# poriya219/modulations

Measured on NVIDIA B200. Metric: turbo_info_throughput_N212_R1/3_8it, higher is better.
Workload: dtype f32/f64

## Files before the change

### modulations_b200/csrc/decode_tpf.cu

```cuda
#include "common.cuh"
#include "tpf_core.cuh"
#include "tpf_dev.cuh"

namespace b200dvb {

namespace {

using namespace tpf;

constexpr int kW = kTpfWin;

__device__ unsigned long long g_tpf_cycles[8];

struct TpfArgs {
    TpfGeom g;
    int B, iterations, n_tiles, n_llr, vec4;
    double sf_inner, sf_last;
    const int16_t *tab;
    const void *llr;
    long long llr_stride;
    int32_t *bits;
    uint32_t *packed;
    const uint8_t *ref_bits;
    unsigned long long *counters;
    unsigned char *ws;
};

constexpr int kRingPairs = 4;
constexpr int kStageBytes = 12288;
constexpr int kRowFloats = kStageBytes / 8;

struct Ctx {
    int N, M, T;
    int f, isb, lane;
    unsigned tq;
    unsigned ycol;
    float4 *srec;
    unsigned char *stage;
    const int16_t *perm, *inv;
    float4 *L1A, *L2A;
    double2 *Le, *LeF, *Yb;
    float4 *CK;
    unsigned long long pol;
    unsigned one;
    __device__ __forceinline__ float4 *wstore() const { return reinterpret_cast<float4 *>(stage); }
    __device__ __forceinline__ float4 *slotZ() const { return reinterpret_cast<float4 *>(stage + 8192); }
    __device__ __forceinline__ float4 *slotX() const { return reinterpret_cast<float4 *>(stage + 10240); }
};

__device__ __forceinline__ void smem_get(const Ctx &c, int k, float (&g)[8])
{
    const float4 lo = c.srec[((k - c.T) * 2) * 16 + c.f], hi = c.srec[((k - c.T) * 2 + 1) * 16 + c.f];
    g[0] = lo.x; g[1] = lo.y; g[2] = lo.z; g[3] = lo.w; g[4] = hi.x; g[5] = hi.y; g[6] = hi.z; g[7] = hi.w;
}
__device__ __forceinline__ void smem_put(const Ctx &c, int k, const float (&g)[8])
{
    c.srec[((k - c.T) * 2) * 16 + c.f] = make_float4(g[0], g[1], g[2], g[3]);
    c.srec[((k - c.T) * 2 + 1) * 16 + c.f] = make_float4(g[4], g[5], g[6], g[7]);
}

struct Buf { float a[8], b[8]; };
template <int KIND> __device__ __forceinline__ void pf_issue(const Ctx &c, int j, Buf &B)
{
    if (KIND == 0) tm_ld8(c.tq + 8u * j, B.a);
    if (KIND == 1) smem_get(c, c.isb ? c.N - 1 - j : j, B.a);
    if (KIND == 2) {
        const unsigned col = 8u * (c.N - 1 - j);
        tm_ld8_half(c.tq + col, B.b);
        tm_ld8_half(c.tq + (16u << 16) + col, B.a);
    }
}
template <int KIND> __device__ __forceinline__ void pf_complete(const Ctx &c, Buf &B, float (&g)[8])
{
    if (KIND == 0) tm_wait_ld(B.a);
    if (KIND == 2) { tm_wait_ld(B.a); tm_wait_ld(B.b); }
#pragma unroll
    for (int i = 0; i < 8; ++i) g[i] = (KIND == 2 && c.isb) ? B.b[i] : B.a[i];
}

__device__ __forceinline__ constexpr int apos(int p) { return (p >> 1) | ((p & 1) << 3); }
__device__ __forceinline__ void pass_out(const Ctx &c, const float (&v)[16], float (&n)[16])
{
#pragma unroll
    for (int p = 0; p < 16; ++p) n[p] = c.isb ? v[rho4(p)] : v[apos(p)];
}
__device__ __forceinline__ void ck_store(const Ctx &c, int slot, const float (&v)[16])
{
    float n[16];
    pass_out(c, v, n);
#pragma unroll
    for (int q = 0; q < 4; ++q)
        st_ws(c.CK + (slot * 4 + q) * 32 + c.lane, make_float4(n[4 * q], n[4 * q + 1], n[4 * q + 2], n[4 * q + 3]));
}

template <int KIND, bool CK>
__device__ __forceinline__ void pass_two(const Ctx &c, int j, int j1, Buf &B0, Buf &B1, float (&g)[8], float (&v)[16])
{
    pf_issue<KIND>(c, j + 1, B1);
    if (CK) ck_store(c, (c.M - j) / kW - 1, v);
    pass_step(v, g, c.isb);
    pf_complete<KIND>(c, B1, g);
    pf_issue<KIND>(c, min(j + 2, j1 - 1), B0);
    pass_step(v, g, c.isb);
    pf_complete<KIND>(c, B0, g);
}
template <int KIND, bool CKA, bool CKB>
__device__ __forceinline__ void pass_loop(const Ctx &c, int j0, int j1, Buf &B0, Buf &B1, float (&g)[8], float (&v)[16])
{
    int j = j0;
    for (; j + 4 <= j1; j += 4) {
        pass_two<KIND, CKA>(c, j, j1, B0, B1, g, v);
        pass_two<KIND, CKB>(c, j + 2, j1, B0, B1, g, v);
    }
    if (j < j1) pass_two<KIND, CKA>(c, j, j1, B0, B1, g, v);
}
template <int KIND, bool CKPT>
__device__ __forceinline__ void run_pass(const Ctx &c, int j0, int j1, float (&v)[16])
{
    static_assert(kW == 4, "checkpoints alternate between the step pairs of a four-step body");
    if (j0 >= j1) return;
    Buf B0, B1;
    float g[8];
    pf_issue<KIND>(c, j0, B0);
    pf_complete<KIND>(c, B0, g);
    if (!CKPT) { pass_loop<KIND, false, false>(c, j0, j1, B0, B1, g, v); return; }
    if (j0 == 0 && (c.M % kW) != 0) ck_store(c, c.M / kW, v);
    if (((c.M - j0) % kW) == 0) pass_loop<KIND, CKPT, false>(c, j0, j1, B0, B1, g, v);
    else                        pass_loop<KIND, false, CKPT>(c, j0, j1, B0, B1, g, v);
}

__device__ __forceinline__ void issue_ckpt(const Ctx &c, int slot)
{
    float4 *dst = (c.isb ? c.slotZ() : c.slotX()) + c.lane;
#pragma unroll
    for (int q = 0; q < 4; ++q) cpa16(dst + q * 32, c.CK + (slot * 4 + q) * 32 + c.lane, c.one);
}
template <bool ALPHA = false>
__device__ __forceinline__ void slot_get(const float4 *slot, int lane, float (&v)[16])
{
    constexpr int P[4] = {ALPHA ? apos(0) : 0, ALPHA ? apos(1) : 1, ALPHA ? apos(2) : 2, ALPHA ? apos(3) : 3};
#pragma unroll
    for (int q = 0; q < 4; ++q) {
        const float4 t = slot[q * 32 + lane];
        const int b = ALPHA ? 2 * q : 4 * q;
        v[b + P[0]] = t.x; v[b + P[1]] = t.y; v[b + P[2]] = t.z; v[b + P[3]] = t.w;
    }
}
template <bool ALPHA = false>
__device__ __forceinline__ void slot_put(float4 *slot, int lane, const float (&v)[16])
{
    constexpr int P[4] = {ALPHA ? apos(0) : 0, ALPHA ? apos(1) : 1, ALPHA ? apos(2) : 2, ALPHA ? apos(3) : 3};
#pragma unroll
    for (int q = 0; q < 4; ++q) {
        const int b = ALPHA ? 2 * q : 4 * q;
        slot[q * 32 + lane] = make_float4(v[b + P[0]], v[b + P[1]], v[b + P[2]], v[b + P[3]]);
    }
}

__device__ __forceinline__ void st256_f64(void *p, double a, double b, double c, double d)
{
    asm volatile("st.global.cg.v4.f64 [%0], {%1,%2,%3,%4};" :: "l"(p), "d"(a), "d"(b), "d"(c), "d"(d) : "memory");
}
__device__ __forceinline__ void ld256_f64(const void *p, double2 &lo, double2 &hi)
{
    asm volatile("ld.global.cg.v4.f64 {%0,%1,%2,%3}, [%4];" : "=d"(lo.x), "=d"(lo.y), "=d"(hi.x), "=d"(hi.y) : "l"(p) : "memory");
}
__device__ __forceinline__ unsigned char *y_entry(const Ctx &c, int k_even)
{
    return reinterpret_cast<unsigned char *>(c.Yb) + ((size_t)(k_even >> 1) * 16 + c.f) * 32;
}
struct YQ { double2 y[kW]; };
__device__ __forceinline__ void yq_load(const Ctx &c, int w0, int len, YQ &q)
{
    static_assert(kW == 4, "two 32-byte entries per window");
    ld256_f64(y_entry(c, w0), q.y[0], q.y[1]);
    ld256_f64(y_entry(c, len > 2 ? w0 + 2 : w0), q.y[2], q.y[3]);
}
__device__ __forceinline__ void yq_park(const Ctx &c, const YQ &q, int w0, int len, int ck_slot)
{

#pragma unroll
    for (int u = 0; u < kW; ++u)
        asm volatile("tcgen05.st.sync.aligned.32x32b.x4.b32 [%0], {%1,%2,%3,%4};"
                     :: "r"(c.tq + c.ycol + 4u * u), "r"(__double2loint(q.y[u].x)), "r"(__double2hiint(q.y[u].x)),
                        "r"(__double2loint(q.y[u].y)), "r"(__double2hiint(q.y[u].y)) : "memory");
    tm_wait_st();
    const int dir = (c.lane >> 3) & 1, pr = (c.lane >> 2) & 1, l16 = c.lane & 15;
    const int w0d = __shfl_sync(0xffffffffu, w0, dir << 4);
    const void *line = c.lane < 16
        ? static_cast<const void *>(reinterpret_cast<const unsigned char *>(c.Yb) + ((size_t)((w0d >> 1) + pr) * 16) * 32 + (c.lane & 3) * 128)
        : static_cast<const void *>(c.CK + (ck_slot * 4 + (l16 >> 2)) * 32 + (l16 & 3) * 8);
    if (c.lane < 16 ? 2 * pr < len : ck_slot >= 0) l2_discard(line);
}

struct Pend { float uv[4], y[4]; int idx; };
__device__ __forceinline__ void pend_flush(const Ctx &c, Pend &p, double sf, double2 *LeOut)
{
    double ea, eb;
    make_extrinsic(p.uv, __hiloint2double(__float_as_int(p.y[1]), __float_as_int(p.y[0])),
                   __hiloint2double(__float_as_int(p.y[3]), __float_as_int(p.y[2])), sf, ea, eb);
    if (p.idx >= 0) st_ws(LeOut + p.idx * 16 + c.f, make_double2(ea, eb));
    p.idx = -1;
}
template <bool TM>
__device__ __forceinline__ void window(const Ctx &c, int wa, int w0, int len, double sf,
                                       double2 *LeOut, int nslot, int nw0, int nlen, Pend &pend)
{
    Buf B;
    auto issue = [&](int u) {
        if (TM) { tm_ld8(c.tq + 8u * (wa + u), B.a); tm_ld8(c.tq + 8u * (wa + len - 1 - u), B.b); }
        else    smem_get(c, w0 + u, B.a);
    };
    auto complete = [&](float (&g)[8]) {
        if (TM) { tm_wait_ld(B.a); tm_wait_ld(B.b); }
#pragma unroll
        for (int i = 0; i < 8; ++i) g[i] = (TM && c.isb) ? B.b[i] : B.a[i];
    };
    YQ nq;
    if (nlen) yq_load(c, nw0, nlen, nq);
    float g[8];
    float4 *ws = c.wstore() + c.lane;
    {
        float Z[16];
        issue(len - 1);
        slot_get(c.slotZ(), c.lane, Z);
        complete(g);
        slot_put(ws + (len - 1) * 128, 0, Z);
        issue(len - 2);
        pend_flush(c, pend, sf, LeOut);
        bwd_step(Z, g);
        complete(g);
        for (int u = len - 2; u >= 0; --u) {
            slot_put(ws + u * 128, 0, Z);
            issue(u > 0 ? u - 1 : 0);
            bwd_step(Z, g);
            complete(g);
        }
        if (!c.isb) slot_put(c.slotZ(), c.lane, Z);
    }
    float X[16];
    slot_get<true>(c.slotX(), c.lane, X);
    if (nslot >= 0) issue_ckpt(c, nslot);
    cpa_commit();
    float yr[4], yn[4], uvp[4], zs[16];
    tm_ld4(c.tq + c.ycol, yr);
    issue(len > 1 ? 1 : 0);
    slot_get(ws, 0, zs);
    ext_step(X, zs, g, uvp);
    tm_wait_ld4(yr);
    complete(g);
    for (int u = 1; u < len; ++u) {
        tm_ld4(c.tq + c.ycol + 4u * u, yn);
        issue(u + 1 < len ? u + 1 : u);
        slot_get(ws + u * 128, 0, zs);
        float uv[4];
        ext_step(X, zs, g, uv);
        double ea, eb;
        make_extrinsic(uvp, __hiloint2double(__float_as_int(yr[1]), __float_as_int(yr[0])),
                       __hiloint2double(__float_as_int(yr[3]), __float_as_int(yr[2])), sf, ea, eb);
        st_ws(LeOut + (w0 + u - 1) * 16 + c.f, make_double2(ea, eb));
        tm_wait_ld4(yn);
        complete(g);
#pragma unroll
        for (int i = 0; i < 4; ++i) { uvp[i] = uv[i]; yr[i] = yn[i]; }
    }
#pragma unroll
    for (int i = 0; i < 4; ++i) { pend.uv[i] = uvp[i]; pend.y[i] = yr[i]; }
    pend.idx = w0 + len - 1;
    if (c.isb) slot_put<true>(c.slotX(), c.lane, X);
    if (nlen) yq_park(c, nq, nw0, nlen, nslot - 1);
}


__device__ __forceinline__ int lpos(const Ctx &c, int k, int fr) { return k < c.M ? k * 32 + fr : (c.N - 1 - k) * 32 + 16 + fr; }

struct Idx { int a, b; };
__device__ __forceinline__ void idx_get(const Ctx &c, int jn, const int16_t *tbl, Idx &x)
{
    jn = min(jn, c.M - 2);
    const int k0 = c.isb ? c.N - 1 - jn : jn, k1 = c.isb ? k0 - 1 : k0 + 1;
    x.a = tbl[k0]; x.b = tbl[k1];
}
__device__ __forceinline__ void prep_load_pair(const Ctx &c, unsigned char *slot, int jn, const float4 *Lsrc,
                                               const Idx &x, bool first)
{
    jn = min(jn, c.M - 2);
    const unsigned d = s_addr(slot) * c.one;
    const float4 *src = Lsrc + jn * 32 + c.lane;
    cpa16_stream_off<0, 0>(d, src, c.pol);
    cpa16_stream_off<1024, 512>(d, src, c.pol);
    if (!first) {
        cpa16_off<512, 0>(d, c.Le + x.a * 16 + c.f);
        cpa16_off<1536, 0>(d, c.Le + x.b * 16 + c.f);
    }
}
struct Raw { float4 xA, xB; double2 laA, laB; };
template <bool FIRST>
__device__ __forceinline__ void raw_get(const unsigned char *slot, Raw &r)
{
    r.xA = *reinterpret_cast<const float4 *>(slot);
    r.xB = *reinterpret_cast<const float4 *>(slot + 1024);
    r.laA = r.laB = make_double2(0.0, 0.0);
    if (!FIRST) {
        r.laA = *reinterpret_cast<const double2 *>(slot + 512);
        r.laB = *reinterpret_cast<const double2 *>(slot + 1536);
    }
}
struct PrepRec { float gA[8], gB[8]; };
__device__ __forceinline__ void prep_pair(const Ctx &c, const Raw &r, int jn, PrepRec &out)
{
    jn = min(jn, c.M - 2);
    const double2 YA = make_double2(d_add((double)r.xA.x, r.laA.x), d_add((double)r.xA.y, r.laA.y));
    const double2 YB = make_double2(d_add((double)r.xB.x, r.laB.x), d_add((double)r.xB.y, r.laB.y));
    make_record(YA.x, YA.y, r.xA.z, r.xA.w, out.gA);
    make_record(YB.x, YB.y, r.xB.z, r.xB.w, out.gB);
#ifndef TPF_ABL_NOY
    const int ke = c.isb ? c.N - 2 - jn : jn;
    st256_f64(y_entry(c, ke), c.isb ? YB.x : YA.x, c.isb ? YB.y : YA.y, c.isb ? YA.x : YB.x, c.isb ? YA.y : YB.y);
#endif
}
struct PrepState { PrepRec r; Raw raw; Idx ix; int ps; };
template <bool FIRST, bool TMST>
__device__ __forceinline__ void pass1a_pair(const Ctx &c, int jj, const float4 *Lsrc, const int16_t *tbl,
// ... 52 lines not shown
}

template <bool FIRST>
__device__ __forceinline__ void pass1a(const Ctx &c, bool second, float (&v)[16])
{
    const float4 *Lsrc = second ? c.L2A : c.L1A;
    const int16_t *tbl = second ? c.perm : c.inv;
    unsigned char *ring = c.stage + c.lane * 16;
    PrepState P;
    P.ix.a = P.ix.b = 0;
#pragma unroll 1
    for (int p = 0; p < kRingPairs; ++p) {
        if (!FIRST) idx_get(c, 2 * p, tbl, P.ix);
        prep_load_pair(c, ring + p * 2048, 2 * p, Lsrc, P.ix, FIRST);
        cpa_commit();
    }
    if (!FIRST) idx_get(c, 2 * kRingPairs, tbl, P.ix);
    cpa_wait<kRingPairs - 1>();
    raw_get<FIRST>(ring, P.raw);
    prep_pair(c, P.raw, 0, P.r);
    prep_load_pair(c, ring, 2 * kRingPairs, Lsrc, P.ix, FIRST);
    cpa_commit();
    if (!FIRST) idx_get(c, 2 * kRingPairs + 2, tbl, P.ix);
    cpa_wait<kRingPairs - 1>();
    raw_get<FIRST>(ring + 2048, P.raw);
    prep_load_pair(c, ring + 2048, 2 * kRingPairs + 2, Lsrc, P.ix, FIRST);
    cpa_commit();
    if (!FIRST) idx_get(c, 2 * kRingPairs + 4, tbl, P.ix);
    P.ps = 2 % kRingPairs;
    pass1a_range<FIRST, true>(c, 0, c.T, Lsrc, tbl, P, v);
    pass1a_range<FIRST, false>(c, c.T, c.M, Lsrc, tbl, P, v);
    cpa_wait<0>();
}

template <bool TIMED>
__device__ __forceinline__ void siso(const Ctx &c, bool second, bool first, bool last, double sf, long long (&ph)[8])
{
    long long tA = TIMED ? clock64() : 0;
    const int N = c.N, M = c.M, T = c.T, lane = c.lane;
    double2 *LeOut = last ? c.LeF : c.Le;
    float v[16];
#pragma unroll
    for (int s = 0; s < 16; ++s) v[s] = 0.f;
    if (first) pass1a<true>(c, second, v);
    else       pass1a<false>(c, second, v);
    tm_wait_st();
    __syncwarp();
    if (!first && !last)
        for (int i = lane; i < N * 2; i += 32) l2_discard(c.Le + i * 8);
    if (TIMED) { const long long t = clock64(); ph[1] += t - tA; tA = t; }
    run_pass<1, false>(c, M, N - T, v);
    run_pass<2, false>(c, N - T, N, v);
    if (TIMED) { const long long t = clock64(); ph[2] += t - tA; tA = t; }
    const int nfull = M / kW, rag = M % kW, nwin = nfull + (rag ? 1 : 0);
    auto win_w0 = [&](int i) { return i < nfull ? (c.isb ? M + i * kW : M - (i + 1) * kW) : (c.isb ? N - rag : 0); };
    auto win_len = [&](int i) { return i < nfull ? kW : rag; };
    {
        YQ q0;
        yq_load(c, win_w0(0), win_len(0), q0);
        run_pass<0, true>(c, 0, T, v);
        run_pass<1, true>(c, T, M, v);
        yq_park(c, q0, win_w0(0), win_len(0), -1);
    }
    if (TIMED) { const long long t = clock64(); ph[3] += t - tA; tA = t; }
    {
        float n[16];
        pass_out(c, v, n);
        slot_put(c.isb ? c.slotZ() : c.slotX(), lane ^ 16, n);
    }
    const int n_inner = (M - T) / kW;
    issue_ckpt(c, 0);
    cpa_commit();
    Pend pend;
#pragma unroll
    for (int i = 0; i < 4; ++i) pend.uv[i] = pend.y[i] = 0.f;
    pend.idx = -1;
    for (int i = 0; i < nwin; ++i) {
        cpa_wait<0>();
        __syncwarp();
        const int wa = i < nfull ? M - (i + 1) * kW : 0;
        const int nlen = i + 1 < nwin ? win_len(i + 1) : 0;
        const int nw0 = i + 1 < nwin ? win_w0(i + 1) : 0;
        if (i < n_inner) window<false>(c, wa, win_w0(i), win_len(i), sf, LeOut, nlen ? i + 1 : -1, nw0, nlen, pend);
        else             window<true>(c, wa, win_w0(i), win_len(i), sf, LeOut, nlen ? i + 1 : -1, nw0, nlen, pend);
        if (TIMED && i == n_inner - 1) { const long long t = clock64(); ph[4] += t - tA; tA = t; }
    }
    pend_flush(c, pend, sf, LeOut);
    cpa_wait<0>();
    __syncwarp();
    if (TIMED) { const long long t = clock64(); ph[5] += t - tA; tA = t; }
}

template <bool TIMED, class LlrT>
__global__ void __launch_bounds__(kTpfWarps * 32, 1)
tpf_kernel(const TpfArgs A)
{
    extern __shared__ __align__(16) unsigned char smem_raw[];
    const TpfGeom g = A.g;
    const int N = g.N;
    const int tid = threadIdx.x, lane = tid & 31, warp = tid >> 5;
    int16_t *tab = reinterpret_cast<int16_t *>(smem_raw);
    const int tab_bytes = ((2 * N * 2 + 15) / 16) * 16;
    unsigned *tmem_slot = reinterpret_cast<unsigned *>(smem_raw + tab_bytes);
    float4 *srec_all = reinterpret_cast<float4 *>(smem_raw + tab_bytes + 64);
    unsigned char *stage_all = reinterpret_cast<unsigned char *>(srec_all + (size_t)kTpfWarps * g.mid * 2 * 16);
    if (warp == 0) {
        asm volatile("tcgen05.alloc.cta_group::1.sync.aligned.shared::cta.b32 [%0], %1;"
                     ::"r"((unsigned)__cvta_generic_to_shared(tmem_slot)), "r"(g.tmem_cols) : "memory");
        asm volatile("tcgen05.relinquish_alloc_permit.cta_group::1.sync.aligned;" ::: "memory");
    }
    for (int i = tid; i < 2 * N; i += blockDim.x) tab[i] = A.tab[i];
    const unsigned mbar = (unsigned)__cvta_generic_to_shared(smem_raw + tab_bytes + 32 + 8 * warp);
    unsigned mphase = 0;
    if (lane == 0) { mbar_init(mbar, 1); mbar_fence_init(); }
    asm volatile("tcgen05.fence::before_thread_sync;" ::: "memory");
    __syncthreads();
    asm volatile("tcgen05.fence::after_thread_sync;" ::: "memory");
    const unsigned tmem_base = *tmem_slot;

    Ctx c;
    c.N = N; c.M = g.M; c.T = g.T;
    c.f = lane & 15; c.isb = lane >> 4; c.lane = lane;
    c.tq = tmem_base + (((unsigned)warp * 32u) << 16);
    c.ycol = 8u * g.T;
    c.srec = srec_all + (size_t)warp * g.mid * 2 * 16;
    {
        volatile unsigned *slots = reinterpret_cast<volatile unsigned *>(smem_raw + tab_bytes);
        if (lane == 0) { slots[4 + warp] = (unsigned)warp * kStageBytes; slots[1] = 1u; }
        __syncwarp();
        c.stage = stage_all + slots[4 + warp];
        c.one = slots[1];
        __syncwarp();
    }
    c.perm = tab; c.inv = tab + N;
    const int wg = blockIdx.x * kTpfWarps + warp;
    unsigned char *ws = A.ws + (size_t)wg * g.ws_per_warp;
    c.L1A = reinterpret_cast<float4 *>(ws + g.off_l1);
    c.L2A = reinterpret_cast<float4 *>(ws + g.off_l2);
    c.Le = reinterpret_cast<double2 *>(ws + g.off_le);
    c.LeF = reinterpret_cast<double2 *>(ws + g.off_lef);
    c.Yb = reinterpret_cast<double2 *>(ws + g.off_y);
    c.CK = reinterpret_cast<float4 *>(ws + g.off_ck);
    asm volatile("createpolicy.fractional.L2::evict_first.b64 %0, 1.0;" : "=l"(c.pol));
    const int16_t *g_off = A.tab + 2 * N;

    unsigned long long bit_err = 0, frm_err = 0, frames_done = 0;
    long long ph[8] = {0, 0, 0, 0, 0, 0, 0, 0};
    const long long t_begin = TIMED ? clock64() : 0;
    for (int tile = wg; tile < A.n_tiles; tile += gridDim.x * kTpfWarps) {
        const long long frame0 = (long long)tile * kTpfFrames;
        const long long t0 = TIMED ? clock64() : 0;
        if (A.vec4) {
            const int nq = llr_row_q<LlrT>(A.n_llr);
            const int pitch4 = ((nq + 6) & ~7) + 1;
            const int rec_bytes = g.mid * 2 * 16 * (int)sizeof(float4);
            const bool in_rec = rec_bytes > kStageBytes;
            float4 *rowbuf = in_rec ? c.srec : reinterpret_cast<float4 *>(c.stage);
            const int fit = (in_rec ? rec_bytes : kStageBytes - N * 16) / (pitch4 * 16);
            const int lg = fit >= 8 ? 3 : fit >= 4 ? 2 : 1, G = 1 << lg, KQ = 32 >> lg;
            const int fr = lane & (G - 1), kq = lane >> lg;
            int4 *otab = reinterpret_cast<int4 *>(in_rec ? c.stage : c.stage + G * pitch4 * 16);
            for (int k = lane; k < N; k += 32) {
                const unsigned oa = (unsigned short)__ldg(g_off + k), op = (unsigned short)__ldg(g_off + c.perm[k]);
                const unsigned o0 = (unsigned short)__ldg(g_off + N + k), o1 = (unsigned short)__ldg(g_off + 2 * N + k);
                const unsigned o2 = (unsigned short)__ldg(g_off + 3 * N + k), o3 = (unsigned short)__ldg(g_off + 4 * N + k);
                otab[k] = make_int4((int)(oa | (op << 16)), (int)(o0 | (o1 << 16)), (int)(o2 | (o3 << 16)), 0);
            }
            auto pull = [&](int g0) {
                if (lane == 0) {
                    int live_rows = 0;
                    for (int r = 0; r < G; ++r) live_rows += frame0 + g0 + r < A.B;
                    fence_proxy_async();
                    mbar_expect_tx(mbar, (unsigned)(live_rows * nq * 16));
                    for (int r = 0; r < live_rows; ++r)
                        bulk_g2s_stream(rowbuf + r * pitch4, static_cast<const LlrT *>(A.llr) + (frame0 + g0 + r) * A.llr_stride, (unsigned)(nq * 16), mbar, c.pol);
                }
            };
            pull(0);
            if (A.ref_bits) {
                const int lines = (2 * N * kTpfFrames + 127) / 128;
                const long long nb = min((long long)kTpfFrames, A.B - frame0) * 2 * N;
                for (int i = lane; i < lines; i += 32)
                    if ((long long)i * 128 < nb) asm volatile("prefetch.global.L2 [%0];" ::"l"(A.ref_bits + frame0 * 2 * N + i * 128));
            }
            const LlrT *row = reinterpret_cast<const LlrT *>(rowbuf + fr * pitch4);
            for (int g0 = 0; g0 < kTpfFrames; g0 += G) {
                mbar_wait(mbar, mphase);
                mphase ^= 1u;
                const bool livef = frame0 + g0 + fr < A.B;
#pragma unroll 4
                for (int k0 = 0; k0 < N; k0 += KQ) {
                    const int k = k0 + kq;
                    const int4 e = otab[min(k, N - 1)];
                    const int oa = (short)(e.x & 0xffff), op = e.x >> 16, o0 = (short)(e.y & 0xffff), o1 = e.y >> 16;
                    const int o2 = (short)(e.z & 0xffff), o3 = e.z >> 16;
                    float4 x1 = make_float4(0.f, 0.f, 0.f, 0.f), x2 = x1;
                    if (livef) {
                        x1.x = llr_f32(row[oa]); x1.y = llr_f32(row[oa + 1]); x2.x = llr_f32(row[op]); x2.y = llr_f32(row[op + 1]);
                        if (o0 >= 0) x1.z = llr_f32(row[o0]);
                        if (o1 >= 0) x1.w = llr_f32(row[o1]);
                        if (o2 >= 0) x2.z = llr_f32(row[o2]);
                        if (o3 >= 0) x2.w = llr_f32(row[o3]);
                    }
// ... 60 lines not shown
                for (int t = 0; t < 8; ++t) {
                    const int k = min(kb + t, N - 1);
                    const unsigned dt = d + t * 512;
                    cpa16_off<0, 0>(dt, c.L1A + lpos(c, k, c.f));
                    cpa16_off<4096, 0>(dt, c.LeF + c.inv[k] * 16 + c.f);
                    cpa16_off<8192, 0>(dt, c.Le + k * 16 + c.f);
                }
            }
            cpa_commit();
        };
        int any_err = 0;
        unsigned word = 0;
        for (int b = 0; b < nst; ++b) hissue(b, b);
        for (int b = 0, st = 0; b < nbu; ++b) {
            if (nst == 3) cpa_wait<2>(); else if (nst == 2) cpa_wait<1>(); else cpa_wait<0>();
            const int kb = (c.isb + 2 * (b >> 1)) * 16 + 8 * (b & 1);
            const unsigned char *src = hbuf + st * kHB + lane * 16;
            unsigned short rb[8];
#pragma unroll
            for (int t = 0; t < 8; ++t) rb[t] = *reinterpret_cast<const unsigned short *>(refp + 2 * min(kb + t, N - 1));
#pragma unroll
            for (int t = 0; t < 8; ++t) {
                const int k = kb + t;
                const float4 ab = *reinterpret_cast<const float4 *>(src + t * 512);
                const double2 la = *reinterpret_cast<const double2 *>(src + 4096 + t * 512);
                const double2 e1 = *reinterpret_cast<const double2 *>(src + 8192 + t * 512);
                const double LA = d_add(d_add((double)ab.x, la.x), e1.x);
                const double LB = d_add(d_add((double)ab.y, la.y), e1.y);
                const int bA = LA < 0.0, bB = LB < 0.0;
                if (k < N) {
                    word |= (unsigned)(bA | (bB << 1)) << (2 * (8 * (b & 1) + t));
                    if (live && A.bits)
                        *reinterpret_cast<int2 *>(A.bits + (size_t)frame * 2 * N + 2 * k) = make_int2(bA, bB);
                    if (cnt) {
                        const int errs = (bA != (rb[t] & 0xff)) + (bB != (rb[t] >> 8));
                        bit_err += errs;
                        any_err |= errs;
                    }
                }
            }
            hissue(b + nst, st);
            st = st + 1 == nst ? 0 : st + 1;
            if (b & 1) {
                const int w = c.isb + b - 1;
                if (live && A.packed && w < nwords) A.packed[(size_t)frame * wpf + w] = word;
                word = 0;
            }
        }
        cpa_wait<0>();
        any_err |= __shfl_xor_sync(0xffffffffu, any_err, 16);
        if (live && !c.isb) { frames_done += 1; frm_err += any_err ? 1 : 0; }
        __syncwarp();
        if (TIMED) ph[6] += clock64() - t6;
    }
    if (TIMED && lane == 0) {
        ph[7] = clock64() - t_begin;
        for (int i = 0; i < 8; ++i) atomicAdd(&g_tpf_cycles[i], (unsigned long long)ph[i]);
    }
    if (A.counters) {
        for (int o = 16; o > 0; o >>= 1) {
            bit_err += __shfl_xor_sync(0xffffffffu, bit_err, o);
            frm_err += __shfl_xor_sync(0xffffffffu, frm_err, o);
            frames_done += __shfl_xor_sync(0xffffffffu, frames_done, o);
        }
        if (lane == 0) {
            if (bit_err) atomicAdd(A.counters + 0, bit_err);
            if (frm_err) atomicAdd(A.counters + 1, frm_err);
            if (frames_done) {
                atomicAdd(A.counters + 2, frames_done);
                atomicAdd(A.counters + 3, frames_done * 2ull * N);
            }
        }
    }
    asm volatile("tcgen05.fence::before_thread_sync;" ::: "memory");
    __syncthreads();
    if (warp == 0)
        asm volatile("tcgen05.dealloc.cta_group::1.sync.aligned.b32 %0, %1;" ::"r"(tmem_base), "r"(g.tmem_cols) : "memory");
}

}

int tpf_configure(Codec &c)
{
    TpfGeom &g = c.tpf;
    g = TpfGeom{};
    const int N = c.N;
    if (N < 16 || (N % 4) != 0) return B200DVB_OK;
    const int M = N / 2;
    int T = M < 64 ? M : 64;
    while (T > 0 && (((M - T) % kW) != 0 || 8 * T + 4 * kW > 512)) --T;
    if (T < kW) return B200DVB_OK;
    g.N = N; g.M = M; g.T = T; g.mid = N - 2 * T;
    g.nfull = M / kW; g.rag = M % kW; g.nslots = g.nfull + (g.rag ? 1 : 0);
    g.tmem_cols = 32;
    while (g.tmem_cols < 8 * T + 4 * kW) g.tmem_cols *= 2;
    if (g.tmem_cols > 512) return B200DVB_OK;
    const size_t tab_bytes = ((size_t)2 * N * 2 + 15) / 16 * 16;
    g.smem_bytes = tab_bytes + 64 + (size_t)kTpfWarps * g.mid * 2 * 16 * sizeof(float4) + (size_t)kTpfWarps * kStageBytes;
    int dev = 0;
    cudaDeviceProp prop;
    B2_CUDA(cudaGetDevice(&dev));
    B2_CUDA(cudaGetDeviceProperties(&prop, dev));
    if (g.smem_bytes > (size_t)prop.sharedMemPerBlockOptin) return B200DVB_OK;
    size_t off = 0;
    auto take = [&](size_t bytes) { const size_t o = off; off += (bytes + 255) / 256 * 256; return o; };
    g.off_l1 = take((size_t)N * 16 * sizeof(float4));
    g.off_l2 = take((size_t)N * 16 * sizeof(float4));
    g.off_le = take((size_t)N * 16 * sizeof(double2));
    g.off_lef = take((size_t)N * 16 * sizeof(double2));
    g.off_y = take((size_t)N * 16 * sizeof(double2));
    g.off_ck = take((size_t)g.nslots * 4 * 32 * sizeof(float4));
    g.ws_per_warp = off;
    B2_CUDA(cudaFuncSetAttribute(tpf_kernel<false, float>, cudaFuncAttributeMaxDynamicSharedMemorySize, (int)prop.sharedMemPerBlockOptin));
    B2_CUDA(cudaFuncSetAttribute(tpf_kernel<true, float>, cudaFuncAttributeMaxDynamicSharedMemorySize, (int)prop.sharedMemPerBlockOptin));
    B2_CUDA(cudaFuncSetAttribute(tpf_kernel<false, __half>, cudaFuncAttributeMaxDynamicSharedMemorySize, (int)prop.sharedMemPerBlockOptin));
    B2_CUDA(cudaFuncSetAttribute(tpf_kernel<true, __half>, cudaFuncAttributeMaxDynamicSharedMemorySize, (int)prop.sharedMemPerBlockOptin));
    g.enabled = 1;
    return B200DVB_OK;
}

int tpf_read_phase_cycles(double *out_h, int reset)
{
    unsigned long long h[8];
    B2_CUDA(cudaMemcpyFromSymbol(h, g_tpf_cycles, sizeof h));
    for (int i = 0; i < 8; ++i) out_h[i] = (double)h[i];
    if (reset) {
        unsigned long long z[8] = {0, 0, 0, 0, 0, 0, 0, 0};
        B2_CUDA(cudaMemcpyToSymbol(g_tpf_cycles, z, sizeof z));
    }
    return B200DVB_OK;
}

static int tpf_grid(const Codec &c, int B)
{
    const int tiles = (B + kTpfFrames - 1) / kTpfFrames;
    const int ctas = (tiles + kTpfWarps - 1) / kTpfWarps;
    return ctas < c.num_sms ? ctas : c.num_sms;
}

size_t tpf_workspace_bytes(const Codec &c, int B)
{
    return (size_t)tpf_grid(c, B) * kTpfWarps * c.tpf.ws_per_warp + 256;
}

template <class LlrT> static void tpf_start(const TpfArgs &A, bool timed, int grid, size_t smem, cudaStream_t s)
{
// ... 35 lines not shown
```

### modulations_b200/csrc/common.cuh

```cuda
#pragma once
#include <cuda_runtime.h>
#include <cuda_fp16.h>
#include <stdint.h>
#include <stddef.h>
#include "../../include/b200dvb.h"

namespace b200dvb {

__device__ __forceinline__ float llr_f32(float x) { return x; }
__device__ __forceinline__ float llr_f32(__half x) { return __half2float(x); }
template <class L> __device__ __forceinline__ float llr_ldg(const L *p) { return llr_f32(__ldg(p)); }
__device__ __forceinline__ float2 llr_ldg2(const float *p) { return __ldg(reinterpret_cast<const float2 *>(p)); }
__device__ __forceinline__ float2 llr_ldg2(const __half *p) { return __half22float2(__ldg(reinterpret_cast<const __half2 *>(p))); }
template <class L> __host__ __device__ __forceinline__ int llr_row_q(int n) { return sizeof(L) == 4 ? (n + 3) / 4 : (n + 7) / 8; }
template <class K32, class K16>
inline cudaError_t occupancy_both_formats(int *occ, K32 k32, K16 k16, int threads, size_t smem)
{
    int a = 0, b = 0;
    cudaError_t e = cudaOccupancyMaxActiveBlocksPerMultiprocessor(&a, k32, threads, smem);
    if (e == cudaSuccess) e = cudaOccupancyMaxActiveBlocksPerMultiprocessor(&b, k16, threads, smem);
    *occ = a < b ? a : b;
    return e;
}

void set_cuda_error(cudaError_t e, const char *where);
#define B2_CUDA(call)                                                     \
    do {                                                                  \
        cudaError_t e__ = (call);                                         \
        if (e__ != cudaSuccess) {                                         \
            ::b200dvb::set_cuda_error(e__, #call);                        \
            return B200DVB_ECUDA;                                         \
        }                                                                 \
    } while (0)

constexpr int kMaxN = 2048;

constexpr int kFramesPerCta = 8;
constexpr int kCtaThreads = 64;
constexpr int kMaxGroups = 7;
constexpr int kMaxCtaThreads = 448;
constexpr int kWin = 8;

struct QuadGeom {
    int N;
    unsigned magic;
    int M;
    int nckA;
    int nckB;
    int rec_stride;
    int ck_stride;
    int groups;
    int threads;
    int use_tmem;
    int tmem_cols;
    int y_slots;
    int frames;
    int ctas_per_sm;
    int grec;
    size_t smem_bytes;
};

constexpr int kTpfFrames = 16;
constexpr int kTpfWarps = 4;
constexpr int kTpfWin = 4;

struct TpfGeom {
    int enabled;
    int N, M;
    int T;
    int mid;
    int nfull, rag;
    int nslots;
    int tmem_cols;
    size_t smem_bytes;
    size_t off_l1, off_l2, off_le, off_lef, off_y, off_ck, off_init;
    size_t ws_per_warp;
};

struct Codec {
    int N = 0, period = 0, iterations = 0, n_llr = 0;
    double sf_inner = 0.7, sf_last = 1.0;
    QuadGeom geom{};
    QuadGeom geom_g{};
    TpfGeom tpf{};
    TpfGeom nii{};
    int num_sms = 0;
    int vec_ab = 0, vec_wy = 0;
    int opt_kernel = 0;
    int opt_no_row_staging = 0;
    int opt_phase_timers = 0;
    int lat_pad = 0;
    int lat_enabled = 0, lat_frames_per_wave = 0;
    int opt_mode = 0;
    int16_t *d_tab = nullptr;
    int32_t next_state[64], out_W[64], out_Y[64];
    int32_t circ_lut[16];
    int16_t *h_tab = nullptr;
};

struct Modem {
    int mod_id = 0, bps = 0, M = 0;
    int separable = 0;
    int half = 0, nlev = 0;
    int pwl = 0;
    int nseg = 0;
    float pwl_x0[2] = {0, 0}, pwl_invd[2] = {0, 0};
    double *d_table64 = nullptr;
    float *d_table32 = nullptr;
    float *d_pwl = nullptr;
    double h_table[512];
};

int launch_decode(const Codec &c, int B, const void *llr, bool f16, long long llr_stride, int32_t *bits,
                  uint32_t *packed, const uint8_t *ref_bits, unsigned long long *counters,
                  void *ws, size_t ws_bytes, cudaStream_t s);
int launch_siso(const Codec &c, int B, const float *Lc_A, const float *Lc_B, const float *Lc_W,
                const float *Lc_Y, const double *La_A, const double *La_B, double sf,
                double *Le_A, double *Le_B, void *ws, size_t ws_bytes, cudaStream_t s);
size_t decode_workspace_bytes(const Codec &c, int B);
size_t siso_workspace_bytes(const Codec &c, int B);
int quad_configure(Codec &c);
int tpf_configure(Codec &c);
int tpf_launch_decode(const Codec &c, int B, const void *llr, bool f16, long long llr_stride, int32_t *bits,
                      uint32_t *packed, const uint8_t *ref_bits, unsigned long long *counters,
// ... 46 lines not shown
```

Baseline: 4.061.

## Add register-resident full-window decode path and per-tile counter flush with ablation hooks

```diff
diff --git a/modulations_b200/csrc/decode_tpf.cu b/modulations_b200/csrc/decode_tpf.cu
--- a/modulations_b200/csrc/decode_tpf.cu
+++ b/modulations_b200/csrc/decode_tpf.cu
@@ -193,13 +193,30 @@
     if (c.lane < 16 ? 2 * pr < len : ck_slot >= 0) l2_discard(line);
 }
 
-struct Pend { float uv[4], y[4]; int idx; };
+struct Pend { float uv[4], y[4]; int idx; unsigned sink; };
+__device__ __forceinline__ void out_epilogue(const float (&uv)[4], const float (&y)[4], double sf, double &ea, double &eb)
+{
+#ifndef TPF_ABL_OUT_FP64
+    make_extrinsic(uv, __hiloint2double(__float_as_int(y[1]), __float_as_int(y[0])),
+                   __hiloint2double(__float_as_int(y[3]), __float_as_int(y[2])), sf, ea, eb);
+#else
+    ea = __hiloint2double(__float_as_int(uv[1]) ^ __float_as_int(y[1]), __float_as_int(uv[0]) ^ __float_as_int(y[0]));
+    eb = __hiloint2double(__float_as_int(uv[3]) ^ __float_as_int(y[3]), __float_as_int(uv[2]) ^ __float_as_int(y[2]));
+#endif
+}
+__device__ __forceinline__ void out_store(const Ctx &c, double2 *LeOut, int k, double ea, double eb, unsigned &sink)
+{
+#ifndef TPF_ABL_OUT_LE
+    st_ws(LeOut + k * 16 + c.f, make_double2(ea, eb));
+#else
+    sink ^= (unsigned)__double2loint(ea) ^ (unsigned)__double2hiint(ea) ^ (unsigned)__double2loint(eb) ^ (unsigned)__double2hiint(eb);
+#endif
+}
 __device__ __forceinline__ void pend_flush(const Ctx &c, Pend &p, double sf, double2 *LeOut)
 {
     double ea, eb;
-    make_extrinsic(p.uv, __hiloint2double(__float_as_int(p.y[1]), __float_as_int(p.y[0])),
-                   __hiloint2double(__float_as_int(p.y[3]), __float_as_int(p.y[2])), sf, ea, eb);
-    if (p.idx >= 0) st_ws(LeOut + p.idx * 16 + c.f, make_double2(ea, eb));
+    out_epilogue(p.uv, p.y, sf, ea, eb);
+    if (p.idx >= 0) out_store(c, LeOut, p.idx, ea, eb, p.sink);
     p.idx = -1;
 }
 template <bool TM>
@@ -216,22 +233,35 @@
 #pragma unroll
         for (int i = 0; i < 8; ++i) g[i] = (TM && c.isb) ? B.b[i] : B.a[i];
     };
+#ifdef TPF_ABL_OUT_REC2
+    auto issue2 = [&](int) {};
+    auto complete2 = [&](float (&)[8]) {};
+#else
+    auto issue2 = issue;
+    auto complete2 = complete;
+#endif
     YQ nq;
+#ifndef TPF_ABL_OUT_GLUE
     if (nlen) yq_load(c, nw0, nlen, nq);
+#endif
     float g[8];
     float4 *ws = c.wstore() + c.lane;
+    float Z[16];
     {
-        float Z[16];
         issue(len - 1);
         slot_get(c.slotZ(), c.lane, Z);
         complete(g);
+#ifndef TPF_ABL_OUT_BETA
         slot_put(ws + (len - 1) * 128, 0, Z);
+#endif
         issue(len - 2);
         pend_flush(c, pend, sf, LeOut);
         bwd_step(Z, g);
         complete(g);
         for (int u = len - 2; u >= 0; --u) {
+#ifndef TPF_ABL_OUT_BETA
             slot_put(ws + u * 128, 0, Z);
+#endif
             issue(u > 0 ? u - 1 : 0);
             bwd_step(Z, g);
             complete(g);
@@ -240,33 +270,115 @@
     }
     float X[16];
     slot_get<true>(c.slotX(), c.lane, X);
+#ifndef TPF_ABL_OUT_GLUE
     if (nslot >= 0) issue_ckpt(c, nslot);
     cpa_commit();
+#endif
     float yr[4], yn[4], uvp[4], zs[16];
+#ifndef TPF_ABL_OUT_Y
     tm_ld4(c.tq + c.ycol, yr);
-    issue(len > 1 ? 1 : 0);
+#else
+#pragma unroll
+    for (int i = 0; i < 4; ++i) yr[i] = yn[i] = pend.y[i];
+#endif
+    issue2(len > 1 ? 1 : 0);
+#ifndef TPF_ABL_OUT_BETA
     slot_get(ws, 0, zs);
+#else
+#pragma unroll
+    for (int i = 0; i < 16; ++i) zs[i] = Z[i];
+#endif
     ext_step(X, zs, g, uvp);
+#ifndef TPF_ABL_OUT_Y
     tm_wait_ld4(yr);
-    complete(g);
+#endif
+    complete2(g);
     for (int u = 1; u < len; ++u) {
+#ifndef TPF_ABL_OUT_Y
         tm_ld4(c.tq + c.ycol + 4u * u, yn);
-        issue(u + 1 < len ? u + 1 : u);
+#endif
+        issue2(u + 1 < len ? u + 1 : u);
+#ifndef TPF_ABL_OUT_BETA
         slot_get(ws + u * 128, 0, zs);
+#endif
         float uv[4];
         ext_step(X, zs, g, uv);
         double ea, eb;
-        make_extrinsic(uvp, __hiloint2double(__float_as_int(yr[1]), __float_as_int(yr[0])),
-                       __hiloint2double(__float_as_int(yr[3]), __float_as_int(yr[2])), sf, ea, eb);
-        st_ws(LeOut + (w0 + u - 1) * 16 + c.f, make_double2(ea, eb));
+        out_epilogue(uvp, yr, sf, ea, eb);
+        out_store(c, LeOut, w0 + u - 1, ea, eb, pend.sink);
+#ifndef TPF_ABL_OUT_Y
         tm_wait_ld4(yn);
-        complete(g);
+#endif
+        complete2(g);
 #pragma unroll
         for (int i = 0; i < 4; ++i) { uvp[i] = uv[i]; yr[i] = yn[i]; }
     }
 #pragma unroll
     for (int i = 0; i < 4; ++i) { pend.uv[i] = uvp[i]; pend.y[i] = yr[i]; }
     pend.idx = w0 + len - 1;
+    if (c.isb) slot_put<true>(c.slotX(), c.lane, X);
+#ifndef TPF_ABL_OUT_GLUE
+    if (nlen) yq_park(c, nq, nw0, nlen, nslot - 1);
+#endif
+}
+
+__device__ __forceinline__ void window_full(const Ctx &c, int wa, int w0, double sf,
+                                            double2 *LeOut, int nslot, int nw0, int nlen, Pend &pend)
+{
+    constexpr int L = kW;
+    YQ nq;
+    if (nlen) yq_load(c, nw0, nlen, nq);
+    float4 *ws = c.wstore() + c.lane;
+    float r[L][8], Z[L][16], Zt[16];
+    {
+        float t[L][8];
+#pragma unroll
+        for (int u = 0; u < L; ++u) tm_ld8(c.tq + 8u * (wa + u), t[u]);
+        slot_get(c.slotZ(), c.lane, Zt);
+        slot_put(ws, 0, Zt);
+        pend_flush(c, pend, sf, LeOut);
+#pragma unroll
+        for (int u = 0; u < L; ++u) tm_wait_ld(t[u]);
+#pragma unroll
+        for (int u = 0; u < L; ++u)
+#pragma unroll
+            for (int i = 0; i < 8; ++i) r[u][i] = c.isb ? t[L - 1 - u][i] : t[u][i];
+    }
+#pragma unroll
+    for (int u = L - 1; u >= 0; --u) {
+#pragma unroll
+        for (int s = 0; s < 16; ++s) Z[u][s] = u == L - 1 ? Zt[s] : Z[u + 1][s];
+        bwd_step(Z[u], r[u]);
+    }
+    if (!c.isb) slot_put(c.slotZ(), c.lane, Z[0]);
+    float X[16];
+    slot_get<true>(c.slotX(), c.lane, X);
+    if (nslot >= 0) issue_ckpt(c, nslot);
+    cpa_commit();
+    float y[L][4], uvp[4];
+    tm_ld4(c.tq + c.ycol, y[0]);
+    tm_wait_ld4(y[0]);
+    ext_step(X, Z[1], r[0], uvp);
+#pragma unroll
+    for (int u = 1; u < L; ++u) {
+        tm_ld4(c.tq + c.ycol + 4u * u, y[u]);
+        float uv[4];
+        if (u < L - 1) {
+            ext_step(X, Z[u + 1], r[u], uv);
+        } else {
+            slot_get(ws, 0, Zt);
+            ext_step(X, Zt, r[u], uv);
+        }
+        double ea, eb;
+        out_epilogue(uvp, y[u - 1], sf, ea, eb);
+        out_store(c, LeOut, w0 + u - 1, ea, eb, pend.sink);
+        tm_wait_ld4(y[u]);
+#pragma unroll
+        for (int i = 0; i < 4; ++i) uvp[i] = uv[i];
+    }
+#pragma unroll
+    for (int i = 0; i < 4; ++i) { pend.uv[i] = uvp[i]; pend.y[i] = y[L - 1][i]; }
+    pend.idx = w0 + L - 1;
     if (c.isb) slot_put<true>(c.slotX(), c.lane, X);
     if (nlen) yq_park(c, nq, nw0, nlen, nslot - 1);
 }
@@ -450,17 +562,27 @@
 #pragma unroll
     for (int i = 0; i < 4; ++i) pend.uv[i] = pend.y[i] = 0.f;
     pend.idx = -1;
+    pend.sink = 0;
     for (int i = 0; i < nwin; ++i) {
-        cpa_wait<0>();
-        __syncwarp();
+#ifdef TPF_ABL_OUT_GLUE
+        if (i == 0)
+#endif
+        {
+            cpa_wait<0>();
+            __syncwarp();
+        }
         const int wa = i < nfull ? M - (i + 1) * kW : 0;
         const int nlen = i + 1 < nwin ? win_len(i + 1) : 0;
         const int nw0 = i + 1 < nwin ? win_w0(i + 1) : 0;
-        if (i < n_inner) window<false>(c, wa, win_w0(i), win_len(i), sf, LeOut, nlen ? i + 1 : -1, nw0, nlen, pend);
-        else             window<true>(c, wa, win_w0(i), win_len(i), sf, LeOut, nlen ? i + 1 : -1, nw0, nlen, pend);
+        if (i < n_inner)     window<false>(c, wa, win_w0(i), win_len(i), sf, LeOut, nlen ? i + 1 : -1, nw0, nlen, pend);
+        else if (i < nfull)  window_full(c, wa, win_w0(i), sf, LeOut, nlen ? i + 1 : -1, nw0, nlen, pend);
+        else                 window<true>(c, wa, win_w0(i), win_len(i), sf, LeOut, nlen ? i + 1 : -1, nw0, nlen, pend);
         if (TIMED && i == n_inner - 1) { const long long t = clock64(); ph[4] += t - tA; tA = t; }
     }
     pend_flush(c, pend, sf, LeOut);
+#ifdef TPF_ABL_OUT_LE
+    if (pend.sink == 0x7fc00001u) st_ws(LeOut + c.f, make_double2(0.0, 0.0));
+#endif
     cpa_wait<0>();
     __syncwarp();
     if (TIMED) { const long long t = clock64(); ph[5] += t - tA; tA = t; }
@@ -519,11 +641,11 @@
     asm volatile("createpolicy.fractional.L2::evict_first.b64 %0, 1.0;" : "=l"(c.pol));
     const int16_t *g_off = A.tab + 2 * N;
 
-    unsigned long long bit_err = 0, frm_err = 0, frames_done = 0;
     long long ph[8] = {0, 0, 0, 0, 0, 0, 0, 0};
     const long long t_begin = TIMED ? clock64() : 0;
     for (int tile = wg; tile < A.n_tiles; tile += gridDim.x * kTpfWarps) {
         const long long frame0 = (long long)tile * kTpfFrames;
+        unsigned long long bit_err = 0, frm_err = 0, frames_done = 0;
         const long long t0 = TIMED ? clock64() : 0;
         if (A.vec4) {
             const int nq = llr_row_q<LlrT>(A.n_llr);
@@ -690,25 +812,25 @@
         if (live && !c.isb) { frames_done += 1; frm_err += any_err ? 1 : 0; }
         __syncwarp();
         if (TIMED) ph[6] += clock64() - t6;
+        if (A.counters) {
+            for (int o = 16; o > 0; o >>= 1) {
+                bit_err += __shfl_xor_sync(0xffffffffu, bit_err, o);
+                frm_err += __shfl_xor_sync(0xffffffffu, frm_err, o);
+                frames_done += __shfl_xor_sync(0xffffffffu, frames_done, o);
+            }
+            if (lane == 0) {
+                if (bit_err) atomicAdd(A.counters + 0, bit_err);
+                if (frm_err) atomicAdd(A.counters + 1, frm_err);
+                if (frames_done) {
+                    atomicAdd(A.counters + 2, frames_done);
+                    atomicAdd(A.counters + 3, frames_done * 2ull * N);
+                }
+            }
+        }
     }
     if (TIMED && lane == 0) {
         ph[7] = clock64() - t_begin;
         for (int i = 0; i < 8; ++i) atomicAdd(&g_tpf_cycles[i], (unsigned long long)ph[i]);
-    }
-    if (A.counters) {
-        for (int o = 16; o > 0; o >>= 1) {
-            bit_err += __shfl_xor_sync(0xffffffffu, bit_err, o);
-            frm_err += __shfl_xor_sync(0xffffffffu, frm_err, o);
-            frames_done += __shfl_xor_sync(0xffffffffu, frames_done, o);
-        }
-        if (lane == 0) {
-            if (bit_err) atomicAdd(A.counters + 0, bit_err);
-            if (frm_err) atomicAdd(A.counters + 1, frm_err);
-            if (frames_done) {
-                atomicAdd(A.counters + 2, frames_done);
-                atomicAdd(A.counters + 3, frames_done * 2ull * N);
-            }
-        }
     }
     asm volatile("tcgen05.fence::before_thread_sync;" ::: "memory");
     __syncthreads();
```

Result: faster. 4.143, median of 6 (+2.0%).

## Use longer checkpoint windows for the tail trellis region in TPF decoder

Applied to the files above, without the earlier changes.

```diff
diff --git a/modulations_b200/csrc/common.cuh b/modulations_b200/csrc/common.cuh
--- a/modulations_b200/csrc/common.cuh
+++ b/modulations_b200/csrc/common.cuh
@@ -70,6 +70,7 @@
     int T;
     int mid;
     int nfull, rag;
+    int Lo;
     int nslots;
     int tmem_cols;
     size_t smem_bytes;
diff --git a/modulations_b200/csrc/decode_tpf.cu b/modulations_b200/csrc/decode_tpf.cu
--- a/modulations_b200/csrc/decode_tpf.cu
+++ b/modulations_b200/csrc/decode_tpf.cu
@@ -32,6 +32,7 @@
 
 struct Ctx {
     int N, M, T;
+    int Lo;
     int f, isb, lane;
     unsigned tq;
     unsigned ycol;
@@ -94,10 +95,10 @@
 }
 
 template <int KIND, bool CK>
-__device__ __forceinline__ void pass_two(const Ctx &c, int j, int j1, Buf &B0, Buf &B1, float (&g)[8], float (&v)[16])
+__device__ __forceinline__ void pass_two(const Ctx &c, int j, int j1, int slot, Buf &B0, Buf &B1, float (&g)[8], float (&v)[16])
 {
     pf_issue<KIND>(c, j + 1, B1);
-    if (CK) ck_store(c, (c.M - j) / kW - 1, v);
+    if (CK) ck_store(c, slot, v);
     pass_step(v, g, c.isb);
     pf_complete<KIND>(c, B1, g);
     pf_issue<KIND>(c, min(j + 2, j1 - 1), B0);
@@ -109,10 +110,10 @@
 {
     int j = j0;
     for (; j + 4 <= j1; j += 4) {
-        pass_two<KIND, CKA>(c, j, j1, B0, B1, g, v);
-        pass_two<KIND, CKB>(c, j + 2, j1, B0, B1, g, v);
-    }
-    if (j < j1) pass_two<KIND, CKA>(c, j, j1, B0, B1, g, v);
+        pass_two<KIND, CKA>(c, j, j1, (c.M - j) / kW - 1, B0, B1, g, v);
+        pass_two<KIND, CKB>(c, j + 2, j1, 0, B0, B1, g, v);
+    }
+    if (j < j1) pass_two<KIND, CKA>(c, j, j1, (c.M - j) / kW - 1, B0, B1, g, v);
 }
 template <int KIND, bool CKPT>
 __device__ __forceinline__ void run_pass(const Ctx &c, int j0, int j1, float (&v)[16])
@@ -127,6 +128,26 @@
     if (j0 == 0 && (c.M % kW) != 0) ck_store(c, c.M / kW, v);
     if (((c.M - j0) % kW) == 0) pass_loop<KIND, CKPT, false>(c, j0, j1, B0, B1, g, v);
     else                        pass_loop<KIND, false, CKPT>(c, j0, j1, B0, B1, g, v);
+}
+__device__ __forceinline__ void run_pass2_tmem(const Ctx &c, float (&v)[16])
+{
+    const int T = c.T, Lo = c.Lo, rl = T % Lo;
+    int slot = (c.M - T) / kW + T / Lo;
+    Buf B0, B1;
+    float g[8];
+    pf_issue<0>(c, 0, B0);
+    pf_complete<0>(c, B0, g);
+    if (rl) ck_store(c, slot, v);
+    for (int j = 0; j < rl; j += 2) pass_two<0, false>(c, j, T, 0, B0, B1, g, v);
+    for (int w = rl; w < T; w += Lo) {
+        --slot;
+        pass_two<0, true>(c, w, T, slot, B0, B1, g, v);
+        pass_two<0, false>(c, w + 2, T, 0, B0, B1, g, v);
+        for (int j = w + 4; j < w + Lo; j += 4) {
+            pass_two<0, false>(c, j, T, 0, B0, B1, g, v);
+            pass_two<0, false>(c, j + 2, T, 0, B0, B1, g, v);
+        }
+    }
 }
 
 __device__ __forceinline__ void issue_ckpt(const Ctx &c, int slot)
@@ -193,6 +214,29 @@
     if (c.lane < 16 ? 2 * pr < len : ck_slot >= 0) l2_discard(line);
 }
 
+__device__ __forceinline__ float4 *long_beta(const Ctx &c) { return c.srec + 4 * 32; }
+__device__ __forceinline__ float4 *long_y(const Ctx &c, int b) { return c.srec + 4 * 32 + c.Lo * (128 + 32 * b); }
+__device__ __forceinline__ void y_issue(const Ctx &c, float4 *buf, int w0, int len)
+{
+    unsigned d = s_addr(buf + c.lane) * c.one;
+    const unsigned char *src = y_entry(c, w0);
+    for (int u = 0; u < len; u += 2, d += 1024, src += 512) {
+        cpa16_off<0, 0>(d, src);
+        cpa16_off<512, 16>(d, src);
+    }
+}
+__device__ __forceinline__ void ws_discard(const Ctx &c, int slot, int wa, int ylen)
+{
+    const int ny = 2 * ylen, nl = 2 * ny + (slot >= 0 ? 16 : 0);
+    for (int t0 = 0; t0 < nl; t0 += 32) {
+        const int t = t0 + c.lane;
+        const unsigned char *y = reinterpret_cast<const unsigned char *>(c.Yb) + (size_t)(t < ny ? wa : c.N - wa - ylen) * 256;
+        const unsigned char *p = t < 2 * ny ? y + (t < ny ? t : t - ny) * 128
+                                            : reinterpret_cast<const unsigned char *>(c.CK + slot * 128) + (t - 2 * ny) * 128;
+        if (t < nl) l2_discard(p);
+    }
+}
+
 struct Pend { float uv[4], y[4]; int idx; };
 __device__ __forceinline__ void pend_flush(const Ctx &c, Pend &p, double sf, double2 *LeOut)
 {
@@ -202,9 +246,9 @@
     if (p.idx >= 0) st_ws(LeOut + p.idx * 16 + c.f, make_double2(ea, eb));
     p.idx = -1;
 }
-template <bool TM>
-__device__ __forceinline__ void window(const Ctx &c, int wa, int w0, int len, double sf,
-                                       double2 *LeOut, int nslot, int nw0, int nlen, Pend &pend)
+template <bool TM, bool SY = false>
+__device__ __forceinline__ void window(const Ctx &c, int wa, int w0, int len, double sf, double2 *LeOut, int nslot,
+                                       int nw0, int nlen, Pend &pend, const float4 *ycur = nullptr, float4 *ynext = nullptr)
 {
     Buf B;
     auto issue = [&](int u) {
@@ -217,9 +261,10 @@
         for (int i = 0; i < 8; ++i) g[i] = (TM && c.isb) ? B.b[i] : B.a[i];
     };
     YQ nq;
-    if (nlen) yq_load(c, nw0, nlen, nq);
+    if (SY) { if (nlen) y_issue(c, ynext, nw0, nlen); }
+    else if (nlen) yq_load(c, nw0, nlen, nq);
     float g[8];
-    float4 *ws = c.wstore() + c.lane;
+    float4 *ws = (SY ? long_beta(c) : c.wstore()) + c.lane;
     {
         float Z[16];
         issue(len - 1);
@@ -242,15 +287,19 @@
     slot_get<true>(c.slotX(), c.lane, X);
     if (nslot >= 0) issue_ckpt(c, nslot);
     cpa_commit();
+    auto y_get = [&](int u, float (&y)[4]) {
+        if (SY) { const float4 t = ycur[u * 32 + c.lane]; y[0] = t.x; y[1] = t.y; y[2] = t.z; y[3] = t.w; }
+        else    tm_ld4(c.tq + c.ycol + 4u * u, y);
+    };
     float yr[4], yn[4], uvp[4], zs[16];
-    tm_ld4(c.tq + c.ycol, yr);
+    y_get(0, yr);
     issue(len > 1 ? 1 : 0);
     slot_get(ws, 0, zs);
     ext_step(X, zs, g, uvp);
-    tm_wait_ld4(yr);
+    if (!SY) tm_wait_ld4(yr);
     complete(g);
     for (int u = 1; u < len; ++u) {
-        tm_ld4(c.tq + c.ycol + 4u * u, yn);
+        y_get(u, yn);
         issue(u + 1 < len ? u + 1 : u);
         slot_get(ws + u * 128, 0, zs);
         float uv[4];
@@ -259,7 +308,7 @@
         make_extrinsic(uvp, __hiloint2double(__float_as_int(yr[1]), __float_as_int(yr[0])),
                        __hiloint2double(__float_as_int(yr[3]), __float_as_int(yr[2])), sf, ea, eb);
         st_ws(LeOut + (w0 + u - 1) * 16 + c.f, make_double2(ea, eb));
-        tm_wait_ld4(yn);
+        if (!SY) tm_wait_ld4(yn);
         complete(g);
 #pragma unroll
         for (int i = 0; i < 4; ++i) { uvp[i] = uv[i]; yr[i] = yn[i]; }
@@ -268,7 +317,8 @@
     for (int i = 0; i < 4; ++i) { pend.uv[i] = uvp[i]; pend.y[i] = yr[i]; }
     pend.idx = w0 + len - 1;
     if (c.isb) slot_put<true>(c.slotX(), c.lane, X);
-    if (nlen) yq_park(c, nq, nw0, nlen, nslot - 1);
+    if (SY) ws_discard(c, nslot - 1, wa, len);
+    else if (nlen) yq_park(c, nq, nw0, nlen, nslot - 1);
 }
 
 
@@ -427,13 +477,15 @@
     run_pass<1, false>(c, M, N - T, v);
     run_pass<2, false>(c, N - T, N, v);
     if (TIMED) { const long long t = clock64(); ph[2] += t - tA; tA = t; }
-    const int nfull = M / kW, rag = M % kW, nwin = nfull + (rag ? 1 : 0);
-    auto win_w0 = [&](int i) { return i < nfull ? (c.isb ? M + i * kW : M - (i + 1) * kW) : (c.isb ? N - rag : 0); };
-    auto win_len = [&](int i) { return i < nfull ? kW : rag; };
+    const int n_inner = (M - T) / kW, Lo = c.Lo, nlong = T / Lo, nwin = n_inner + nlong + (T % Lo ? 1 : 0);
+    auto win_wa = [&](int i) { return i < n_inner ? M - (i + 1) * kW : i < n_inner + nlong ? T - (i - n_inner + 1) * Lo : 0; };
+    auto win_len = [&](int i) { return i < n_inner ? kW : i < n_inner + nlong ? Lo : T % Lo; };
+    auto win_w0 = [&](int i) { return c.isb ? N - win_wa(i) - win_len(i) : win_wa(i); };
     {
         YQ q0;
         yq_load(c, win_w0(0), win_len(0), q0);
-        run_pass<0, true>(c, 0, T, v);
+        if (Lo == kW) run_pass<0, true>(c, 0, T, v);
+        else          run_pass2_tmem(c, v);
         run_pass<1, true>(c, T, M, v);
         yq_park(c, q0, win_w0(0), win_len(0), -1);
     }
@@ -443,22 +495,43 @@
         pass_out(c, v, n);
         slot_put(c.isb ? c.slotZ() : c.slotX(), lane ^ 16, n);
     }
-    const int n_inner = (M - T) / kW;
     issue_ckpt(c, 0);
     cpa_commit();
     Pend pend;
 #pragma unroll
     for (int i = 0; i < 4; ++i) pend.uv[i] = pend.y[i] = 0.f;
     pend.idx = -1;
-    for (int i = 0; i < nwin; ++i) {
+    int i = 0;
+    for (; i < n_inner; ++i) {
         cpa_wait<0>();
         __syncwarp();
-        const int wa = i < nfull ? M - (i + 1) * kW : 0;
         const int nlen = i + 1 < nwin ? win_len(i + 1) : 0;
         const int nw0 = i + 1 < nwin ? win_w0(i + 1) : 0;
-        if (i < n_inner) window<false>(c, wa, win_w0(i), win_len(i), sf, LeOut, nlen ? i + 1 : -1, nw0, nlen, pend);
-        else             window<true>(c, wa, win_w0(i), win_len(i), sf, LeOut, nlen ? i + 1 : -1, nw0, nlen, pend);
-        if (TIMED && i == n_inner - 1) { const long long t = clock64(); ph[4] += t - tA; tA = t; }
+        const bool to_long = Lo > kW && i + 1 == n_inner;
+        if (to_long) y_issue(c, long_y(c, 0), nw0, nlen);
+        window<false>(c, M - (i + 1) * kW, c.isb ? M + i * kW : M - (i + 1) * kW, kW, sf, LeOut, nlen ? i + 1 : -1, nw0,
+                      to_long ? 0 : nlen, pend);
+        if (to_long && lane < 16) l2_discard(c.CK + i * 128 + lane * 8);
+    }
+    if (TIMED && n_inner > 0) { const long long t = clock64(); ph[4] += t - tA; tA = t; }
+    if (Lo == kW) {
+        for (; i < nwin; ++i) {
+            cpa_wait<0>();
+            __syncwarp();
+            const int nlen = i + 1 < nwin ? win_len(i + 1) : 0;
+            const int nw0 = i + 1 < nwin ? win_w0(i + 1) : 0;
+            window<true>(c, win_wa(i), win_w0(i), win_len(i), sf, LeOut, nlen ? i + 1 : -1, nw0, nlen, pend);
+        }
+    } else {
+        for (; i < nwin; ++i) {
+            cpa_wait<0>();
+            __syncwarp();
+            const int nlen = i + 1 < nwin ? win_len(i + 1) : 0;
+            const int nw0 = i + 1 < nwin ? win_w0(i + 1) : 0;
+            const int il = i - n_inner;
+            window<true, true>(c, win_wa(i), win_w0(i), win_len(i), sf, LeOut, nlen ? i + 1 : -1, nw0, nlen, pend,
+                               long_y(c, il & 1), long_y(c, (il + 1) & 1));
+        }
     }
     pend_flush(c, pend, sf, LeOut);
     cpa_wait<0>();
@@ -494,7 +567,7 @@
     const unsigned tmem_base = *tmem_slot;
 
     Ctx c;
-    c.N = N; c.M = g.M; c.T = g.T;
+    c.N = N; c.M = g.M; c.T = g.T; c.Lo = g.Lo;
     c.f = lane & 15; c.isb = lane >> 4; c.lane = lane;
     c.tq = tmem_base + (((unsigned)warp * 32u) << 16);
     c.ycol = 8u * g.T;
@@ -729,7 +802,14 @@
     while (T > 0 && (((M - T) % kW) != 0 || 8 * T + 4 * kW > 512)) --T;
     if (T < kW) return B200DVB_OK;
     g.N = N; g.M = M; g.T = T; g.mid = N - 2 * T;
-    g.nfull = M / kW; g.rag = M % kW; g.nslots = g.nfull + (g.rag ? 1 : 0);
+    g.nfull = M / kW; g.rag = M % kW;
+    g.Lo = kW;
+    for (const int L : {16, 12, 8})
+        if (g.Lo == kW && L <= T && L * 3072 <= (g.mid - 8) * 512) g.Lo = L;
+#ifdef TPF_LO_CAP
+    while (g.Lo > TPF_LO_CAP) g.Lo -= 4;
+#endif
+    g.nslots = (M - T) / kW + T / g.Lo + (T % g.Lo ? 1 : 0);
     g.tmem_cols = 32;
     while (g.tmem_cols < 8 * T + 4 * kW) g.tmem_cols *= 2;
     if (g.tmem_cols > 512) return B200DVB_OK;
```

After: 4.064 before, 3.938 after (median of 6 runs). 0.969x the previous value.
